# cyrillefavreau/Sol-R

Hardware: AMD Instinct MI355X
Metric: Mrays/s @1920x1080, 3-bounce Cornell (higher is better)
Workload: dtype f32; 1 GPU; cornell 1920x1080, 3 bounces + shadow rays, 75 boxes / 29 primitives, one GPU, whole frame; rays_per_frame=6518779, closest_hit_walks_rank0=3506171, lane_nodes=206382796, lane_prim_tests=37557299, wave_nodes=3396811, wave_prim_tests=626627, wave_walks=106204, cost_ordered_launch_rank0=True, frames_in_flight=3, setup_frames_before_warmup=48, frames_delivered=9105, order_free_nodes=46, short_ray_lists=1, gather=none (one GPU), strips=equal rows, parallelism=tile1

## Files before the change

sol-r_amd/csrc/engine.h:

```cpp
#ifndef SOLR_ENGINE_H
#define SOLR_ENGINE_H

#include <hip/hip_runtime.h>

#include <atomic>
#include <chrono>
#include <cstdio>
#include <cstdlib>
#include <cstring>
#include <string>
#include <utility>
#include <vector>

#include "../../include/solr_hip.h"
#include "renderer.h"
#include "lists_device.h"
#include "list_builders.h"

namespace solreng
{
struct HostProfile
{
    const bool on = getenv("SOLR_HIP_HOST_PROFILE") != nullptr;
    struct Entry
// ... 184 lines not shown
    VARIANT_AUTOMATIC = 0,
    VARIANT_EXACT_LIST = 3,
    VARIANT_ALL_FEATURES = 4,
    VARIANT_NO_GROUPING = 5,
    VARIANT_NO_ORDER_FREE = 6,
    VARIANT_STACK_IN_LDS = 7,
    VARIANT_REFERENCE_LEAVES = 8,
    VARIANT_AO_FIXED_STRIDE = 9,
    VARIANT_NAN_DEEP_STACK = 10,
    VARIANT_UNSORTED_LISTS = 12,
    VARIANT_NO_BAND_WORDS = 13,
    VARIANT_ZERO_STREAM_COUNTERS = 14,
    VARIANT_NO_LAMP_CUTOFF = 15,
    VARIANT_ALL_TRIPS = 16,
    VARIANT_UPLOADED_BUILD_BOXES = 17,
    VARIANT_UPLOADED_SPHERE_LEAVES = 18
};

__host__ __device__ inline int primitiveKind(int type, int facts)
{
    if (!(facts & PRIM_FAST0))
        return KIND_GENERAL;
    if (type == ptSphere && !(facts & PRIM_PROCEDURAL))
        return KIND_SPHERE;
    if ((type == ptXYPlane || type == ptYZPlane || type == ptXZPlane) && !(facts & (PRIM_TEXTURED | PRIM_WIRE2)) &&
        !(type == ptYZPlane && (facts & PRIM_EMISSIVE)))
        return type == ptXYPlane ? KIND_PLANE_XY : (type == ptYZPlane ? KIND_PLANE_YZ : KIND_PLANE_XZ);
    if (type == ptTriangle)
        return KIND_TRIANGLE;
    if (type == ptCylinder || type == ptCone)
        return KIND_CYLINDER;
// ... 33 lines not shown
        return features | F_PLANE;
    }
}

struct NodeList
{
    int copies, lists;
    explicit NodeList(int copies_ = 1, int lists_ = 1) : copies(copies_), lists(lists_) {}
    std::vector<float4> rows;
    std::vector<int> start, origin;
    int nb = 0;
    unsigned offRows = 0, offLeaf = 0;
    unsigned offStart = 0;
    int ordered = 0;
    bool tight = false;
    std::vector<int> refitLevels;

    void reset() { *this = NodeList(copies, lists); }
    unsigned nodes() const { return (unsigned)lists * (unsigned)nb; }
    unsigned rowsOf(int list) const { return solrdev::listRows(offRows, (unsigned)nb, (unsigned)list); }
    unsigned offThin() const { return solrdev::listThin(offRows, nodes()); }
    unsigned offSorted() const { return solrdev::listSorted(offRows, nodes()); }
    unsigned layRows(unsigned row)
    {
        offRows = row;
        return row + (unsigned)copies * solrdev::listCopyRows(nodes());
    }
    unsigned layStart(unsigned row)
    {
        offStart = row * 4;
        return row + (nodes() + 3u) / 4u;
    }
    unsigned layLeaf(unsigned row)
    {
        row = (row + 3u) & ~3u;
        offLeaf = row;
        return row + 4u * nodes() + 4u;
// ... 69 lines not shown
    int slotA, slotB;
    bool moves;
};
struct Morph
{
    MorphKey keys[MORPH_SLOTS];
    int nbTrackKeys = 0;
    std::vector<MorphLampAnswer> lampAnswers;
    long lampChecked = -1;
    DeviceBuffer lampFlag;
    int nbDeviceMorphs = 0;
    int nbDeviceTrackMorphs = 0;
};
struct Scene
{
    NodeList exact = NodeList(1, 1), walk = NodeList(2, 1), orderFree = NodeList(3, solrdev::ORDER_FREE_LISTS);
    std::vector<float4> hostPrims;
    int nbPrimitives = 0;
    DeviceBuffer lamps;
    int nbLamps = 0;
    int nested = 1;
    bool walkEncloses = false;
    OrderFreeState lists;
    Rotation rotation;
    Morph morph;
    long retags = 0;
    Arena arena;

    struct Served
    {
        int rotations, translations, lampMoves, edits, materialSets, morphs, trackMorphs;
// ... 559 lines not shown
void h2dMaterialsOne(Material *materials, int nbActiveMaterials);
MaterialRecord materialRecord(const Material &material, int i, solrdev::MaterialHot &hot, solrdev::MaterialCold &cold);
void h2dRandomsOne(float *randoms);
void h2dRandomsSizedOne(const float *randoms, long count);
void h2dTexturesOne(int activeTextures, TextureInfo *textureInfos);
void h2dLightInformationOne(LightInformation *lightInformation, int lightInformationSize);
void setMovableOne(const unsigned char *flags, int nbPrimitives);
void retagPrimitives();
void checkTextureTables();
void maybeBuildOrderFreeLists();
void flushGeometry();
void pullGeometry();
void ensureHostFreeLists();
void buildLeafRecords();
void tightenListsAgain();
float thinReachWanted(float viewDistance);
bool listEnclosesInArena(const NodeList &list);
ListKnobs listKnobs();
PruneDecider pruneDecider();
bool orderFreeListsUsable();
bool lampCutoffUsable();
bool shortRayListsChoice();
SceneArgs prepareScene(const SceneInfo &sceneInfo, bool exactNodes);
bool deepNodeList(const SceneArgs &S);
bool canRotateOne(const float center[3], const float cosAngles[3], const float sinAngles[3], float viewDistance,
                  const char *who = "solr_hip_rotate_primitives");
int rotatePrimitivesOne(const float center[3], const float cosAngles[3], const float sinAngles[3], float viewDistance);
bool refitMovedScene(float viewDistance);
void refreshExactList();
int setMorphKeysOne(const Primitive *first, const Primitive *last, int nbPrimitives);
// ... 75 lines not shown
```

sol-r_amd/csrc/renderer_kernel.h:

```cpp
#ifndef SOLR_RENDERER_KERNEL_H
#define SOLR_RENDERER_KERNEL_H

#include "renderer.h"

using namespace solrdev;

template <int COUNT, int FEAT, bool VOLUME = false>
#ifndef SOLR_GENERIC_WAVES
#define SOLR_GENERIC_WAVES 0
#endif
#ifndef SOLR_WAVES_PER_EU
#define SOLR_WAVES_PER_EU 4
#endif
__global__ __launch_bounds__(WAVE, (SOLR_GENERIC_WAVES && (FEAT & F_TEX)) ? SOLR_GENERIC_WAVES : SOLR_WAVES_PER_EU) void k_standardRenderer(const SceneArgs, const FrameArgs,
                                                           PixelRecord *__restrict__,
                                                           int4 *__restrict__, unsigned char *__restrict__,
                                                           unsigned long long *__restrict__)
{
    extern __shared__ float ldsStack[];
    constexpr int ARGS = FEAT | F_ARGS;
    constexpr int TRACE = (FEAT & (F_TRI | F_TEX)) ? FEAT : ARGS;
    const RendererArgs &A = rendererArgs();
    const FrameArgs &F = A.F;
    const Scene &S = A.scene();
// ... 402 lines not shown
    for (int j = 0; j < walks; ++j)
    {
        const int4 h = head[1 + j];
        const int kind = __builtin_amdgcn_readfirstlane(h.x);
        if (kind == WALK_GENERAL)
        {
            ++left_out;
            continue;
        }
        const float4 a = rays[((size_t)j * 64 + lane) * 2], b = rays[((size_t)j * 64 + lane) * 2 + 1];
        const int doneAfter = __float_as_int(b.w);
        const bool took_part = doneAfter >= 0;
        const WalkRay r = makeWalkRay(V(a.x, a.y, a.z), took_part ? V(b.x, b.y, b.z) : V(1.f, 1.f, 1.f));
        const int order = (FEAT & F_DEEP) ? (__builtin_amdgcn_readfirstlane(h.w) >> 1) & 3 : 0;
        const Scene W = walkList(S, __builtin_amdgcn_readfirstlane(h.y) != 0, __builtin_amdgcn_readfirstlane(h.z),
                                 (__builtin_amdgcn_readfirstlane(h.w) & 1) != 0, order != 0);
        const PackedRay pr = packRay(r);
        const float cutOff = a.w;
        int cursor = took_part ? 0 : SOLR_CURSOR_DONE;
        int cur = 0, visit = 0;
        while (cur < W.nbBoxes)
        {
            if (ballot(cursor != SOLR_CURSOR_DONE) == 0ull)
                break;
            int nbPrimitives;
            bool entered;
            int leaf;
            if ((FEAT & F_DEEP) && order == 1)
                leaf = advanceTidyDeepSorted(W, pr, cutOff, cursor, cur, nbPrimitives, entered);
            else if ((FEAT & F_DEEP) && order == 2)
                leaf = advanceTidyDeepReversed(W, pr, cutOff, cursor, cur, nbPrimitives, entered);
// ... 17 lines not shown
```

sol-r_amd/csrc/rt_device.h:

```cpp
#pragma once

#include <hip/hip_runtime.h>
#include "pow_table.h"

#include "../../include/solr_types.h"
#include "scene_layout.h"

namespace solrdev
{
#define SOLR_DEV __device__ __forceinline__

struct v3
{
    float x, y, z;
};

SOLR_DEV v3 V(float x, float y, float z)
{
    v3 r;
    r.x = x;
    r.y = y;
    r.z = z;
    return r;
}
// ... 856 lines not shown
    }
    return v;
}

#define SOLR_CURSOR_DONE 0x7fffffff

#define SOLR_WALK_SLOTS 16
#define SOLR_WALK_SLOT_BYTES (16 * (SOLR_WALK_SLOTS + 1) + SOLR_WALK_SLOTS * 64 * 32)
enum WalkKind
{
    WALK_CLOSEST = 0,
    WALK_SHADOW = 1,
    WALK_GENERAL = 2
};
SOLR_DEV void recordWalk(Counters &cnt, int kind, bool freeList, int octant, bool took_part, const WalkRay &r, float cutOff,
                         int doneAfter, bool tight = false, int order = 0)
{
    const unsigned j = cnt.ordinal++;
    if (j >= SOLR_WALK_SLOTS || !cnt.record)
        return;
    const int lane = (int)threadIdx.x & 63;
    float4 *lanes = (float4 *)(cnt.record + 16 * (SOLR_WALK_SLOTS + 1)) + ((size_t)j * 64 + lane) * 2;
    lanes[0] = make_float4(r.o.x, r.o.y, r.o.z, cutOff);
    lanes[1] = make_float4(r.d.x, r.d.y, r.d.z, __int_as_float(took_part ? doneAfter : -1));
    if (lane == 0)
        ((int4 *)cnt.record)[1 + j] = make_int4(kind, freeList ? 1 : 0, octant, (tight ? 1 : 0) | (order << 1));
}

template <int FEAT>
SOLR_DEV bool extendedGeometry(const SceneInfo &si);
struct PrimRec
{
    Row2 head;
    float4 c, d;
    int pi;
    bool packed;
};
SOLR_DEV bool planeClass(int type)
{
    return !(type == ptSphere || type == ptEnvironment || type == ptCylinder || type == ptCone || type == ptEllipsoid ||
             type == ptTriangle);
// ... 812 lines not shown
    int octant = 0;
    bool reversed = false;
    if (freeOrder)
    {
        const int signs = ((r.d.x < 0.f ? 1 : 0) | (r.d.y < 0.f ? 2 : 0) | (r.d.z < 0.f ? 4 : 0)) ^ 7;
        const int lane = (int)__builtin_ctzll(ballot(active));
        octant = __builtin_amdgcn_readlane(signs, lane);
        reversed = (FEAT & F_DEEP) && S.sortedLists && ballot(active && signs != octant) == 0ull;
    }
    if (freeOrder || lampCut)
        farFree = 1.0002f + 1.0e-4f * (fabsf(r.o.x) + fabsf(r.o.y) + fabsf(r.o.z)) / lengthOL;
    const float farOrdered =
        (lampCut && longRay(r.d) && minDistance >= 2.f) ? fminf(minDistance, farFree) : minDistance;
    const bool tight = (FEAT & F_PLANE) && tidy && S.tightLists && ballot(active && !tightRay(r, si)) == 0ull;
    reversed = reversed && !tight;
    const Scene W = walkList(S, freeOrder, octant, tight, reversed);
    const int nbBoxes = W.nbBoxes;
    const PackedRay pr = packRay(r);
    int cursor = (active && result < si.shadowIntensity) ? 0 : SOLR_CURSOR_DONE;
    const bool walked = cursor != SOLR_CURSOR_DONE;
    int visit = 0, doneAfter = SOLR_CURSOR_DONE;
    int cur = 0;
    Row2 node;
    node.a = node.b = make_float4(0.f, 0.f, 0.f, 0.f);
    if (!tidy)
        node = boxNode(S, 0);
    while (cur < nbBoxes)
    {
        if (ballot(cursor != SOLR_CURSOR_DONE) == 0ull)
            break;
        int leaf = cur, nbPrimitives;
// ... 131 lines not shown
                }
            }
        }
        if (COUNT == 2)
            ++visit;
        if (cursor != SOLR_CURSOR_DONE && !(result < si.shadowIntensity))
        {
            cursor = SOLR_CURSOR_DONE;
            if (COUNT == 2)
                doneAfter = visit;
        }
        SOLR_T(cnt.tLeaf += SOLR_NOW() - ta; ++cnt.nLeaf;)
    }
    if (COUNT == 2)
        recordWalk(cnt, tidy ? WALK_SHADOW : WALK_GENERAL, freeOrder, octant, walked, r, freeOrder ? farFree : farOrdered,
                   doneAfter, tight, reversed ? 2 : 0);
    result = fmaxf(0.f, fminf(result, si.shadowIntensity));
    SOLR_T(cnt.tShadow += SOLR_NOW() - tw0;)
    return result;
}


SOLR_DEV float rnd(const Scene &S, long i)
{
    return (i >= 0 && i < S.nbRandoms) ? S.randoms[i] : 0.f;
}

template <int FEAT>
SOLR_DEV float4 intersectionShader(const Scene &S, const SceneInfo &si, int pi, int type, int materialId,
                                   const MaterialHot &mh, v3 intersection, v3 areas, const TexOut &o)
{
// ... 979 lines not shown
```

sol-r_amd/csrc/scene_layout.h:

```cpp
#pragma once

#include <hip/hip_runtime.h>

namespace solrdev
{
struct alignas(16) MaterialHot
{
    float4 innerIllumination;
    float4 color;
    float4 specular;
    float reflection, refraction, transparency, opacity;
    int4 attributes;
    int4 ids;
};
static_assert(sizeof(MaterialHot) == 96, "MaterialHot");

struct alignas(16) MaterialCold
{
    int4 textureMapping;
    int4 textureOffset;
    int4 textureIds;
    int4 advancedTextureOffset;
    int4 advancedTextureIds;
    float2 mappingOffset;
// ... 42 lines not shown
    ROW_SIZE_MAT = 1,
    ROW_P1_INDEX = 2,
    ROW_P2 = 3,
    ROW_N0 = 4,
    ROW_N1 = 5,
    ROW_N2 = 6,
    ROW_UV = 7,
    PRIM_ROWS = 8
};

enum ShadowFacts
{
    SHADOWS_OPAQUE = 1,
    SHADOWS_LAMP_CUTOFF = 2,
    SHADOWS_ALL_TRIPS = 4
};

struct SceneArgs
{
    const void *geometry;
    const void *materials;
    const void *textures;
    const void *randoms;
    unsigned offBoxes, offBoxStart, offPrims, offLights, offMatCold;
    int nbBoxes;
    int nbPrimitives;
    int nbLights;
    int nbLamps;
    int nested;
    int orderedBoxes;
    long nbRandoms;
    unsigned offLeaf;
    unsigned offBoxesFree, offLeafFree;
    int nbBoxesFree;
    int opaqueShadows;
    int shortRayLists;
    int tightLists;
    int sortedLists;
};

const int ORDER_FREE_LISTS = 8;
__host__ __device__ constexpr unsigned listCopyRows(unsigned nodes) { return 2u * nodes + 2u; }
__host__ __device__ constexpr unsigned listRows(unsigned offRows, unsigned nb, unsigned list) { return offRows + 2u * (list * nb); }
__host__ __device__ constexpr unsigned listThin(unsigned offRows, unsigned nodes) { return offRows + listCopyRows(nodes); }
__host__ __device__ constexpr unsigned listSorted(unsigned offRows, unsigned nodes) { return offRows + 2u * listCopyRows(nodes); }
__host__ __device__ constexpr unsigned listLeaf(unsigned offLeaf, unsigned nb, unsigned list) { return offLeaf + 4u * (list * nb); }

#define SOLR_CONST_AS __attribute__((address_space(4)))
typedef float f4v __attribute__((ext_vector_type(4)));
typedef int i4v __attribute__((ext_vector_type(4)));
typedef const SOLR_CONST_AS f4v *cf4p;
typedef const SOLR_CONST_AS i4v *ci4p;
typedef const SOLR_CONST_AS int *cip;
typedef const SOLR_CONST_AS float *cfp;
typedef const SOLR_CONST_AS unsigned char *cbp;

struct Scene
{
    cf4p geo;
    cf4p mat;
// ... 34 lines not shown
    s.nbLamps = a.nbLamps;
    s.nested = a.nested;
    s.orderedBoxes = a.orderedBoxes;
    s.nbRandoms = a.nbRandoms;
    s.offLeaf = a.offLeaf;
    s.offBoxesFree = a.offBoxesFree;
    s.offLeafFree = a.offLeafFree;
    s.nbBoxesFree = a.nbBoxesFree;
    s.opaqueShadows = a.opaqueShadows;
    s.shortRayLists = a.shortRayLists;
    s.tightLists = a.tightLists;
    s.sortedLists = a.sortedLists;
    return s;
}

__device__ __forceinline__ Scene walkList(const Scene &S, bool freeList, int octant, bool thin, bool sorted)
{
    Scene W = S;
    unsigned nodes = (unsigned)S.nbBoxes;
    if (freeList)
    {
        nodes = (unsigned)ORDER_FREE_LISTS * (unsigned)S.nbBoxesFree;
        W.offBoxes = listRows(S.offBoxesFree, (unsigned)S.nbBoxesFree, (unsigned)octant);
        W.offLeaf = listLeaf(S.offLeafFree, (unsigned)S.nbBoxesFree, (unsigned)octant);
        W.nbBoxes = S.nbBoxesFree;
    }
    if (freeList && sorted)
    {
        W.offBoxes = listSorted(W.offBoxes, nodes);
        W.nbBoxes = S.nbBoxesFree << 5;
    }
    else if (thin)
        W.offBoxes = listThin(W.offBoxes, nodes);
    return W;
}

typedef float f8v __attribute__((ext_vector_type(8)));
typedef const SOLR_CONST_AS f8v *cf8p;
typedef const SOLR_CONST_AS char *ccp;

__device__ __forceinline__ float4 ld4(cf4p p, unsigned row)
{
    const f4v v = *(cf4p)((ccp)p + (row << 4));
    return make_float4(v.x, v.y, v.z, v.w);
}
struct Row2
{
    float4 a, b;
// ... 88 lines not shown
```

sol-r_amd/csrc/solr_arena.hip:

```cpp
#include <hip/hip_runtime.h>

#include <cmath>

#include "../../include/solr_hip.h"
#include "rt_device.h"

using namespace solrdev;

#include "renderer.h"
#include "engine.h"

using namespace solreng;

namespace solreng
{
__global__ __launch_bounds__(256) void k_buildLeafRecords(float4 *__restrict__ arena, unsigned offNodes, unsigned offStart,
                                                         unsigned offPrims, unsigned offLeaf, int nbNodes)
{
    const int i = blockIdx.x * blockDim.x + threadIdx.x;
    if (i >= nbNodes)
        return;
    float4 r0 = make_float4(0.f, 0.f, 0.f, 0.f), r1 = r0, r2 = r0, r3 = r0;
    const int nb = __float_as_int(arena[offNodes + 2u * (unsigned)i + 1u].z);
    if (nb > 0)
// ... 59 lines not shown
    for (int j = i + 1; j < end; ++j)
    {
        const float4 b = arena[offTight + 2u * (unsigned)j + 1u];
        if (__float_as_int(b.z) <= 0)
            continue;
        const float4 a = arena[offTight + 2u * (unsigned)j];
        lx = fminf(lx, a.x), ly = fminf(ly, a.y), lz = fminf(lz, a.z);
        hx = fmaxf(hx, b.x), hy = fmaxf(hy, b.y), hz = fmaxf(hz, a.w);
    }
    const float nlx = fmaxf(row0.x, lx), nly = fmaxf(row0.y, ly), nlz = fmaxf(row0.z, lz);
    const float nhx = fminf(row1.x, hx), nhy = fminf(row1.y, hy), nhz = fminf(row0.w, hz);
    if (!(nlx <= nhx && nly <= nhy && nlz <= nhz))
        return;
    arena[offTight + 2u * (unsigned)i] = make_float4(nlx, nly, nlz, nhz);
    arena[offTight + 2u * (unsigned)i + 1u] = make_float4(nhx, nhy, row1.z, row1.w);
}

__global__ __launch_bounds__(256) void k_listEncloses(const float4 *__restrict__ arena, unsigned offNodes, unsigned offStart,
                                                      unsigned offPrims, int nbNodes, int nbPrims, int *bad)
{
    const int i = blockIdx.x * blockDim.x + threadIdx.x;
    if (i >= nbNodes)
        return;
    const float4 a = arena[offNodes + 2u * (unsigned)i], b = arena[offNodes + 2u * (unsigned)i + 1u];
    const int count = __float_as_int(b.z);
    const int end = min(i + max(__float_as_int(b.w), 1), nbNodes);
    bool encloses = true;
    if (count <= 0)
    {
        for (int j = i + 1; j < end && encloses;)
// ... 105 lines not shown
    static const bool off = getenv("SOLR_HIP_NO_TIGHT_LEAVES") != nullptr;
    const int nbNodes = (int)list.nodes(), listLength = list.nb;
    const bool worth = g.facts.plainPlanes || (g.facts.looseSpheres && (g.facts.sceneFeatures & F_PLANE) != 0);
    if (off || !worth || nbNodes <= 0 || listLength <= 0 || listLength > 65536 || !ok())
        return false;
    float4 *arena = (float4 *)g.scene.arena.geometry.ptr;
    const float margin = g.facts.sceneExtent * (1.f / 1024.f);
    const dim3 grid((unsigned)((nbNodes + 255) / 256));
    hipLaunchKernelGGL(k_tightenLeaves, grid, dim3(256), 0, sceneStream(), arena, list.offRows, list.offThin(), list.offStart, g.scene.arena.offPrims,
                       nbNodes, margin, g.facts.thinReach);
    hipLaunchKernelGGL(k_tightenInner, grid, dim3(256), 0, sceneStream(), arena, list.offThin(), nbNodes, listLength);
    HIPCHECK(hipGetLastError());
    return ok();
}

__global__ __launch_bounds__(256) void k_sortNodeBounds(float4 *__restrict__ arena, unsigned offBoxesFree, unsigned offSorted, int nb)
{
    const int i = blockIdx.x * blockDim.x + threadIdx.x;
    if (i > 8 * nb)
        return;
    float4 a = make_float4(0.f, 0.f, 0.f, 0.f), b = a;
    if (i < 8 * nb)
    {
        const int octant = i / nb;
        a = arena[offBoxesFree + 2u * (unsigned)i];
        b = arena[offBoxesFree + 2u * (unsigned)i + 1u];
        if (octant & 1)
        {
            const float t = a.x;
            a.x = b.x;
// ... 26 lines not shown
    hipLaunchKernelGGL(k_sortNodeBounds, dim3((unsigned)((8 * list.nb + 1 + 255) / 256)), dim3(256), 0, sceneStream(),
                       (float4 *)g.scene.arena.geometry.ptr, list.offRows, list.offSorted(), list.nb);
    HIPCHECK(hipGetLastError());
    return ok();
}

static void deriveList(NodeList &list)
{
    const bool orderFree = &list == &g.scene.orderFree;
    const int n = (orderFree && g.scene.lists.freeStale) ? 0 : (int)list.nodes();
    if (n > 0)
        hipLaunchKernelGGL(k_buildLeafRecords, dim3((unsigned)((n + 255) / 256)), dim3(256), 0, sceneStream(), (float4 *)g.scene.arena.geometry.ptr,
                           list.offRows, list.offStart, g.scene.arena.offPrims, list.offLeaf, n);
    HIPCHECK(hipGetLastError());
    list.tight = list.copies > 1 && n > 0 && tightenList(list);
    if (orderFree)
        g.scene.lists.sortedFree = n > 0 && sortFreeLists();
}

void buildLeafRecords()
{
    if (!ok() || !g.scene.arena.geometry.ptr)
        return;
    for (NodeList *list : {&g.scene.exact, &g.scene.walk, &g.scene.orderFree})
        deriveList(*list);
    HIPCHECK(hipStreamSynchronize(sceneStream()));
}

void tightenListsAgain()
{
    if (!ok() || !g.scene.arena.geometry.ptr)
        return;
    for (NodeList *list : {&g.scene.walk, &g.scene.orderFree})
        if (list->tight)
            list->tight = tightenList(*list);
    HIPCHECK(hipStreamSynchronize(sceneStream()));
}

static void copyStagedLists()
{
    const NodeList &list = g.scene.orderFree;
    char *arena = (char *)g.scene.arena.geometry.ptr;
    const SolrDeviceLists &stage = g.scene.lists.freeStage;
    HIPCHECK(hipMemcpyAsync(arena + (size_t)list.offRows * 16, stage.rows, (size_t)list.nodes() * 32, hipMemcpyDeviceToDevice, sceneStream()));
    HIPCHECK(hipMemcpyAsync(arena + (size_t)list.offStart * 4, stage.start, (size_t)list.nodes() * 4, hipMemcpyDeviceToDevice, sceneStream()));
}

static void appendFreeLists()
{
    const unsigned end = g.scene.orderFree.layLeaf(g.scene.orderFree.layStart(g.scene.orderFree.layRows(g.scene.arena.rowsFixed)));
// ... 210 lines not shown
    return g.scene.orderFree.nb > 0 && g.facts.primsContained && !g.scene.lists.freeStale && g.scene.nested && g.scene.walk.ordered &&
           g.variant != VARIANT_NO_ORDER_FREE;
}

bool lampCutoffUsable()
{
    return g.scene.walkEncloses && g.facts.primsContained && g.scene.nested && g.scene.walk.ordered && g.variant != VARIANT_NO_LAMP_CUTOFF;
}

static int tightListsFor(const SceneArgs &S, const SceneInfo &sceneInfo, bool exactNodes)
{
    if (exactNodes || g.variant == VARIANT_REFERENCE_LEAVES || !g.scene.walk.tight || !g.scene.walkEncloses || !sceneInfo.extendedGeometry)
        return 0;
    if (S.nbBoxesFree > 0 && !g.scene.orderFree.tight)
        return 0;
    return (sceneInfo.viewDistance > 0.f && sceneInfo.viewDistance <= 64.f * g.facts.sceneExtent) ? 1 : 0;
}

static bool sortedListsUsable(int nbBoxesFree)
{
    return nbBoxesFree > 0 && g.scene.lists.sortedFree && g.variant != VARIANT_UNSORTED_LISTS;
}

bool shortRayListsChoice()
{
    static const int fromEnv = getenv("SOLR_HIP_SHORT_RAY_LISTS") ? atoi(getenv("SOLR_HIP_SHORT_RAY_LISTS")) : -1;
    const int mode = g.shortRayListsMode >= 0 ? g.shortRayListsMode : fromEnv;
    return mode < 0 ? activeFlights() >= 2 : mode != 0;
}

static SceneArgs makeScene(bool exactNodes)
// ... 67 lines not shown
```

sol-r_amd/csrc/solr_diag.hip:

```cpp
#include <hip/hip_runtime.h>
#include <dlfcn.h>
#include <fcntl.h>
#include <sched.h>
#include <sys/mman.h>
#include <sys/stat.h>
#include <unistd.h>

#include <atomic>

#include <cmath>
#include <cstdio>
#include <cstdlib>
#include <cstring>
#include <string>
#include <functional>
#include <chrono>
#include <vector>

#include "../../include/solr_hip.h"
#include "rt_device.h"
#include "device_pool.h"
#include "lists_device.h"

using namespace solrdev;
// ... 61 lines not shown
    }
    HIPCHECK(hipMemcpyAsync(bitmapOut, bitmap, pixels * SOLR_COLOR_DEPTH, hipMemcpyDeviceToHost, stream));
    HIPCHECK(hipStreamSynchronize(stream));
    return ok() ? 0 : -1;
}

void lastFrame(int out[6])
{
    memcpy(out, g.lastFrame, sizeof(g.lastFrame));
}

int listCopy(int list, int what, void *out, int capacity)
{
    if (!ready("solr_hip_probe_list_copy"))
        return -1;
    ARGCHECK(list >= 0 && list <= 2 && what >= 0 && what <= 4, "solr_hip_probe_list_copy: no such list or copy");
    ARGCHECK(g.scene.arena.geometry.ptr != nullptr || g.scene.arena.geometryDirty, "solr_hip_probe_list_copy: no scene uploaded");
    if (!ok())
        return -1;
    HIPCHECK(hipSetDevice(g.device));
    flushGeometry();
    if (list == 1)
        refreshExactList();
    quiesce();
    if (!ok() || !g.scene.arena.geometry.ptr)
        return -1;
    const NodeList &L = list == 0 ? g.scene.walk : (list == 1 ? g.scene.exact : g.scene.orderFree);
    const unsigned nodes = (list == 2 && g.scene.lists.freeStale) ? 0u : L.nodes();
    size_t at = 0, count = 0, unit = 16;
    switch (what)
    {
    case 0:
        at = (size_t)L.offRows * 16, count = 2 * (size_t)nodes;
        break;
    case 1:
        at = (size_t)L.offThin() * 16, count = (L.copies > 1 && L.tight) ? 2 * (size_t)nodes : 0;
        break;
    case 2:
        at = (size_t)L.offSorted() * 16, count = (list == 2 && L.copies > 2 && g.scene.lists.sortedFree) ? 2 * (size_t)nodes + 2 : 0;
        break;
    case 3:
        at = (size_t)L.offLeaf * 16, count = 4 * (size_t)nodes;
        break;
    default:
        at = (size_t)L.offStart * 4, count = nodes, unit = 4;
        break;
    }
    if (nodes == 0)
        count = 0;
    if (!out)
        return (int)count;
    ARGCHECK(count <= (size_t)(capacity < 0 ? 0 : capacity), "solr_hip_probe_list_copy: capacity too small");
    ARGCHECK(at + count * unit <= g.scene.arena.geometry.bytes, "solr_hip_probe_list_copy: the copy lies outside the arena");
    if (!ok())
        return -1;
    if (count)
        HIPCHECK(hipMemcpy(out, (const char *)g.scene.arena.geometry.ptr + at, count * unit, hipMemcpyDeviceToHost));
    return ok() ? (int)count : -1;
}

int walkOffer(const SceneInfo &sceneInfo, bool exactNodes, int out[8])
{
    SceneArgs S;
    int features, deep;
    hipStream_t stream;
    if (residentScene(sceneInfo, exactNodes, &S, &features, &deep, &stream) != 0)
        return -1;
    const float margin = g.facts.sceneExtent * (1.f / 1024.f), extent = g.facts.sceneExtent;
    out[0] = S.tightLists, out[1] = S.sortedLists, out[2] = S.nbBoxesFree, out[3] = S.opaqueShadows, out[4] = S.shortRayLists;
    out[5] = S.nbBoxes;
    memcpy(&out[6], &margin, 4);
    memcpy(&out[7], &extent, 4);
    return 0;
}
}

extern "C" {
static unsigned long long walkLists[6];
void solr_hip_walk_bound_lists(unsigned long long out[6])
{
    if (out)
        memcpy(out, walkLists, sizeof(walkLists));
}

// ... 393 lines not shown
```

sol-r_amd/csrc/solr_materials.hip:

```cpp
#include <hip/hip_runtime.h>

#include "../../include/solr_hip.h"
#include "rt_device.h"

using namespace solrdev;

#include "renderer.h"
#include "engine.h"

using namespace solreng;

namespace solreng
{
__global__ __launch_bounds__(256) void k_setPrimitiveMaterials(float4 *__restrict__ arena, unsigned offPrims, int nbPrimitives,
                                                               const int4 *__restrict__ batch, int nbRecords, int noKinds)
{
    const int e = blockIdx.x * blockDim.x + threadIdx.x;
    if (e >= nbRecords)
        return;
    const int4 r = batch[e];
    const int slot = r.x;
    if (slot < 0 || slot >= nbPrimitives)
        return;
    float4 *rows = arena + offPrims + (size_t)PRIM_ROWS * slot;
// ... 121 lines not shown
    HIPCHECK(hipMemcpyAsync(g.scene.rotation.materialSets.ptr, batch.data(), batch.size() * sizeof(int4), hipMemcpyHostToDevice, sceneStream()));
    hipLaunchKernelGGL(k_setPrimitiveMaterials, dim3((unsigned)((n + 255) / 256)), dim3(256), 0, sceneStream(),
                       (float4 *)g.scene.arena.geometry.ptr, g.scene.arena.offPrims, g.scene.nbPrimitives,
                       (const int4 *)g.scene.rotation.materialSets.ptr, n, general ? 1 : 0);
    LeafMaterialsFollow M;
    const int nodes = leafRecordsOfLists(g.scene, M.list);
    M.offPrims = g.scene.arena.offPrims;
    M.nbPrimitives = g.scene.nbPrimitives;
    if (nodes > 0)
        hipLaunchKernelGGL(k_followLeafRecords, dim3((unsigned)((nodes + 255) / 256)), dim3(256), 0, sceneStream(),
                           (float4 *)g.scene.arena.geometry.ptr, M);
    HIPCHECK(hipGetLastError());
    HIPCHECK(hipStreamSynchronize(sceneStream()));
    if (ok())
    {
        for (int i = 0; i < n; ++i)
        {
            float4 *r = &g.scene.hostPrims[(size_t)PRIM_ROWS * slots[i]];
            const int tag = bitsi(r[ROW_P0_TYPE].w), type = tag & PRIM_TYPE_MASK, facts = batch[(size_t)i].z;
            g.facts.count(type, factsOfTag(tag), -1);
            g.facts.count(type, facts, +1);
            r[ROW_P0_TYPE].w = bitsf(primitiveTag(type, facts, general));
            r[ROW_SIZE_MAT].w = bitsf(materialIds[i]);
            r[ROW_P2].w = bitsf(batch[(size_t)i].w);
        }
        g.facts.deriveFromCounts();
        g.scene.retagged();
    }
    g.scene.materialSetsServed(ok());
    return ok() ? 1 : 0;
}

enum
{
    RETAG_LINEAR = 8
};
__global__ __launch_bounds__(256) void k_retagMaterials(float4 *__restrict__ arena, unsigned offPrims, int nbPrimitives,
                                                        const int4 *__restrict__ batch, int nbRecords, int noKinds)
{
    const int p = blockIdx.x * blockDim.x + threadIdx.x;
    if (p >= nbPrimitives)
        return;
// ... 171 lines not shown
                               (const int4 *)M.editBatch.ptr, (int)plan.batch.size(), general ? 1 : 0);
            LeafMaterialsFollow F;
            const int nodes = leafRecordsOfLists(g.scene, F.list);
            F.offPrims = g.scene.arena.offPrims;
            F.nbPrimitives = g.scene.nbPrimitives;
            if (nodes > 0)
                hipLaunchKernelGGL(k_followLeafRecords, dim3((unsigned)((nodes + 255) / 256)), dim3(256), 0, sceneStream(),
                                   (float4 *)g.scene.arena.geometry.ptr, F);
            HIPCHECK(hipGetLastError());
        }
    }
    HIPCHECK(hipStreamSynchronize(sceneStream()));
    M.nbImaged = ok() ? M.nbImaged : -1;
    if (!ok())
        return 0;
    for (size_t k = 0; k < plan.ids.size(); ++k)
    {
        const size_t id = (size_t)plan.ids[k];
        M.imageHot[id] = plan.hot[k];
        M.imageCold[id] = plan.cold[k];
        M.materialTags[id] = plan.records[k].facts;
        M.materialAverage[id] = plan.records[k].average;
    }
    std::vector<TextureUse> uses;
    size_t k = 0;
    for (const TextureUse &use : M.textureUses)
    {
        for (; k < plan.ids.size() && plan.ids[k] < use.material; ++k)
            if (plan.records[k].textured)
                uses.push_back(plan.records[k].use);
// ... 14 lines not shown
            changedAt[(size_t)plan.batch[e].x] = (int)e;
        for (int p = 0; p < g.scene.nbPrimitives; ++p)
        {
            float4 *r = &g.scene.hostPrims[(size_t)PRIM_ROWS * p];
            const int material = bitsi(r[ROW_SIZE_MAT].w);
            if (material < 0 || material >= M.nbImaged || changedAt[(size_t)material] < 0)
                continue;
            const int4 &record = plan.batch[(size_t)changedAt[(size_t)material]];
            r[ROW_P0_TYPE].w = bitsf(primitiveTag(bitsi(r[ROW_P0_TYPE].w) & PRIM_TYPE_MASK, record.y, general));
            r[ROW_P2].w = bitsf(record.z);
        }
        g.facts = plan.after;
        g.scene.retagged();
        ++M.nbDeviceRetags;
    }
    ++M.nbDeviceEdits;
    return 1;
}

}

extern "C" {
int solr_hip_device_material_sets(void)
{
    return g.scene.rotation.nbDeviceMaterialSets;
}
int solr_hip_device_material_edits(void)
{
    return g.materials.nbDeviceEdits;
}
// ... 6 lines not shown
```

sol-r_amd/csrc/solr_probes.hip:

```cpp
#include <hip/hip_runtime.h>

#include <cstdio>
#include <cstring>
#include <string>
#include <vector>

#include "../../include/solr_hip.h"
#include "../../include/solr_hip_probes.h"
#include "../../include/solr_hip_probes_morph.h"
#include "rt_device.h"
#include "renderer.h"
#include "list_builders.h"
#include "lists_device.h"

using namespace solrdev;

namespace solrprobe
{
int residentScene(const SceneInfo &sceneInfo, bool exactNodes, SceneArgs *S, int *features, int *deepList, hipStream_t *stream);
void fail(int code, const char *what);
int ticketOfSerial(long long serial, int *slot, long long *period);
long long imageSerial(long long setTo);
int postProcess(const SceneInfo &sceneInfo, const PostProcessingInfo &ppInfo, const PostProcessingBuffer *frame,
                unsigned char *bitmapOut);
// ... 205 lines not shown
    const int e = blockIdx.x * 64 + threadIdx.x;
    const bool active = e < n;
    const int q = active ? e : 0;
    Counters cnt;
    memset(&cnt, 0, sizeof(cnt));
    float value = 0.f;
    v3 tint = V(0.f, 0.f, 0.f);
    unsigned long long todo = ballot(active);
    while (todo)
    {
        const int first = (int)__builtin_ctzll(todo);
        const int lamp = __builtin_amdgcn_readlane(lightId[q], first);
        const int it = __builtin_amdgcn_readlane(iteration[q], first);
        const bool lanes = active && lightId[q] == lamp && iteration[q] == it;
        v3 c = V(0.f, 0.f, 0.f);
        const float s = shadowWalk<false, FEAT>(S, si, lanes, at3(lampCenters, q), at3(origins, q), lamp, it, c, objectId[q], cnt);
        if (lanes)
        {
            value = s;
            tint = c;
        }
        todo &= ~ballot(lanes);
    }
    if (active)
    {
        result[e] = value;
        put3(color, e, tint);
    }
}

template <int FEAT>
// ... 741 lines not shown
```

Measured before the change: 31600 Mrays/s.

## Add shadow-specific thin BVH copy that culls lamp-only and non-fast leaves

Builds a third copy of the walk node list for shadow rays. Leaves whose primitives are all non-FAST0 or are the single lamp itself get an unenterable corner box, and inner bounds are re-tightened over the remaining leaves. Shadow walks select this copy through a new TIGHT_SHADOW_COPY bit, which is meant to avoid node and primitive tests that cannot occlude. The cost is extra arena rows, two build kernels, a rebuild whenever materials change FAST0, and added correctness complexity around lamp identity.

```diff
diff --git a/sol-r_amd/csrc/engine.h b/sol-r_amd/csrc/engine.h
--- a/sol-r_amd/csrc/engine.h
+++ b/sol-r_amd/csrc/engine.h
@@ -222,7 +222,8 @@
     VARIANT_NO_LAMP_CUTOFF = 15,
     VARIANT_ALL_TRIPS = 16,
     VARIANT_UPLOADED_BUILD_BOXES = 17,
-    VARIANT_UPLOADED_SPHERE_LEAVES = 18
+    VARIANT_UPLOADED_SPHERE_LEAVES = 18,
+    VARIANT_THIN_SHADOW_WALKS = 19
 };
 
 __host__ __device__ inline int primitiveKind(int type, int facts)
@@ -286,6 +287,7 @@
     unsigned offStart = 0;
     int ordered = 0;
     bool tight = false;
+    bool shadow = false;
     std::vector<int> refitLevels;
 
     void reset() { *this = NodeList(copies, lists); }
@@ -293,6 +295,7 @@
     unsigned rowsOf(int list) const { return solrdev::listRows(offRows, (unsigned)nb, (unsigned)list); }
     unsigned offThin() const { return solrdev::listThin(offRows, nodes()); }
     unsigned offSorted() const { return solrdev::listSorted(offRows, nodes()); }
+    unsigned offShadow() const { return solrdev::listShadow(offRows, nodes()); }
     unsigned layRows(unsigned row)
     {
         offRows = row;
@@ -392,7 +395,7 @@
 };
 struct Scene
 {
-    NodeList exact = NodeList(1, 1), walk = NodeList(2, 1), orderFree = NodeList(3, solrdev::ORDER_FREE_LISTS);
+    NodeList exact = NodeList(1, 1), walk = NodeList(3, 1), orderFree = NodeList(3, solrdev::ORDER_FREE_LISTS);
     std::vector<float4> hostPrims;
     int nbPrimitives = 0;
     DeviceBuffer lamps;
@@ -982,6 +985,7 @@
 void ensureHostFreeLists();
 void buildLeafRecords();
 void tightenListsAgain();
+void shadowListAgain();
 float thinReachWanted(float viewDistance);
 bool listEnclosesInArena(const NodeList &list);
 ListKnobs listKnobs();
diff --git a/sol-r_amd/csrc/renderer_kernel.h b/sol-r_amd/csrc/renderer_kernel.h
--- a/sol-r_amd/csrc/renderer_kernel.h
+++ b/sol-r_amd/csrc/renderer_kernel.h
@@ -440,7 +440,8 @@
         const WalkRay r = makeWalkRay(V(a.x, a.y, a.z), took_part ? V(b.x, b.y, b.z) : V(1.f, 1.f, 1.f));
         const int order = (FEAT & F_DEEP) ? (__builtin_amdgcn_readfirstlane(h.w) >> 1) & 3 : 0;
         const Scene W = walkList(S, __builtin_amdgcn_readfirstlane(h.y) != 0, __builtin_amdgcn_readfirstlane(h.z),
-                                 (__builtin_amdgcn_readfirstlane(h.w) & 1) != 0, order != 0);
+                                 (__builtin_amdgcn_readfirstlane(h.w) & 1) != 0, order != 0,
+                                 (__builtin_amdgcn_readfirstlane(h.w) & 8) != 0 ? 2u : 1u);
         const PackedRay pr = packRay(r);
         const float cutOff = a.w;
         int cursor = took_part ? 0 : SOLR_CURSOR_DONE;
diff --git a/sol-r_amd/csrc/rt_device.h b/sol-r_amd/csrc/rt_device.h
--- a/sol-r_amd/csrc/rt_device.h
+++ b/sol-r_amd/csrc/rt_device.h
@@ -894,7 +894,7 @@
     WALK_GENERAL = 2
 };
 SOLR_DEV void recordWalk(Counters &cnt, int kind, bool freeList, int octant, bool took_part, const WalkRay &r, float cutOff,
-                         int doneAfter, bool tight = false, int order = 0)
+                         int doneAfter, bool tight = false, int order = 0, bool shadowCopy = false)
 {
     const unsigned j = cnt.ordinal++;
     if (j >= SOLR_WALK_SLOTS || !cnt.record)
@@ -904,7 +904,7 @@
     lanes[0] = make_float4(r.o.x, r.o.y, r.o.z, cutOff);
     lanes[1] = make_float4(r.d.x, r.d.y, r.d.z, __int_as_float(took_part ? doneAfter : -1));
     if (lane == 0)
-        ((int4 *)cnt.record)[1 + j] = make_int4(kind, freeList ? 1 : 0, octant, (tight ? 1 : 0) | (order << 1));
+        ((int4 *)cnt.record)[1 + j] = make_int4(kind, freeList ? 1 : 0, octant, (tight ? 1 : 0) | (order << 1) | (shadowCopy ? 8 : 0));
 }
 
 template <int FEAT>
@@ -1747,7 +1747,8 @@
         (lampCut && longRay(r.d) && minDistance >= 2.f) ? fminf(minDistance, farFree) : minDistance;
     const bool tight = (FEAT & F_PLANE) && tidy && S.tightLists && ballot(active && !tightRay(r, si)) == 0ull;
     reversed = reversed && !tight;
-    const Scene W = walkList(S, freeOrder, octant, tight, reversed);
+    const unsigned thinCopy = (FEAT & F_PLANE) ? ((unsigned)S.tightLists + 1u) >> 1 : 1u;
+    const Scene W = walkList(S, freeOrder, octant, tight, reversed, thinCopy);
     const int nbBoxes = W.nbBoxes;
     const PackedRay pr = packRay(r);
     int cursor = (active && result < si.shadowIntensity) ? 0 : SOLR_CURSOR_DONE;
@@ -1909,7 +1910,7 @@
     }
     if (COUNT == 2)
         recordWalk(cnt, tidy ? WALK_SHADOW : WALK_GENERAL, freeOrder, octant, walked, r, freeOrder ? farFree : farOrdered,
-                   doneAfter, tight, reversed ? 2 : 0);
+                   doneAfter, tight, reversed ? 2 : 0, tight && !freeOrder && thinCopy == 2u);
     result = fmaxf(0.f, fminf(result, si.shadowIntensity));
     SOLR_T(cnt.tShadow += SOLR_NOW() - tw0;)
     return result;
diff --git a/sol-r_amd/csrc/scene_layout.h b/sol-r_amd/csrc/scene_layout.h
--- a/sol-r_amd/csrc/scene_layout.h
+++ b/sol-r_amd/csrc/scene_layout.h
@@ -80,6 +80,12 @@
     SHADOWS_OPAQUE = 1,
     SHADOWS_LAMP_CUTOFF = 2,
     SHADOWS_ALL_TRIPS = 4
+};
+
+enum TightLists
+{
+    TIGHT_LISTS = 1,
+    TIGHT_SHADOW_COPY = 2
 };
 
 struct SceneArgs
@@ -110,6 +116,8 @@
 __host__ __device__ constexpr unsigned listRows(unsigned offRows, unsigned nb, unsigned list) { return offRows + 2u * (list * nb); }
 __host__ __device__ constexpr unsigned listThin(unsigned offRows, unsigned nodes) { return offRows + listCopyRows(nodes); }
 __host__ __device__ constexpr unsigned listSorted(unsigned offRows, unsigned nodes) { return offRows + 2u * listCopyRows(nodes); }
+__host__ __device__ constexpr unsigned listShadow(unsigned offRows, unsigned nodes) { return offRows + 2u * listCopyRows(nodes); }
+#define SOLR_UNENTERABLE_CORNER 0x1p100f
 __host__ __device__ constexpr unsigned listLeaf(unsigned offLeaf, unsigned nb, unsigned list) { return offLeaf + 4u * (list * nb); }
 
 #define SOLR_CONST_AS __attribute__((address_space(4)))
@@ -174,7 +182,7 @@
     return s;
 }
 
-__device__ __forceinline__ Scene walkList(const Scene &S, bool freeList, int octant, bool thin, bool sorted)
+__device__ __forceinline__ Scene walkList(const Scene &S, bool freeList, int octant, bool thin, bool sorted, unsigned thinCopy = 1u)
 {
     Scene W = S;
     unsigned nodes = (unsigned)S.nbBoxes;
@@ -191,7 +199,7 @@
         W.nbBoxes = S.nbBoxesFree << 5;
     }
     else if (thin)
-        W.offBoxes = listThin(W.offBoxes, nodes);
+        W.offBoxes += (freeList ? 1u : thinCopy) * listCopyRows(nodes);
     return W;
 }
 
diff --git a/sol-r_amd/csrc/solr_arena.hip b/sol-r_amd/csrc/solr_arena.hip
--- a/sol-r_amd/csrc/solr_arena.hip
+++ b/sol-r_amd/csrc/solr_arena.hip
@@ -97,6 +97,85 @@
         return;
     arena[offTight + 2u * (unsigned)i] = make_float4(nlx, nly, nlz, nhz);
     arena[offTight + 2u * (unsigned)i + 1u] = make_float4(nhx, nhy, row1.z, row1.w);
+}
+
+__device__ __forceinline__ bool unenterable(const float4 &row0, const float4 &row1)
+{
+    const float c = SOLR_UNENTERABLE_CORNER;
+    return row0.x == c && row0.y == c && row0.z == c && row0.w == c && row1.x == c && row1.y == c;
+}
+__global__ __launch_bounds__(256) void k_shadowLeaves(float4 *__restrict__ arena, unsigned offThin, unsigned offShadow, unsigned offStart,
+                                                     unsigned offPrims, unsigned offLights, int nbNodes, int nbPrims, int nbLamps,
+                                                     int nbLights)
+{
+    const int i = blockIdx.x * blockDim.x + threadIdx.x;
+    if (i >= nbNodes)
+        return;
+    float4 row0 = arena[offThin + 2u * (unsigned)i], row1 = arena[offThin + 2u * (unsigned)i + 1u];
+    const int nb = __float_as_int(row1.z);
+    if (nb > 0)
+    {
+        bool oneLamp = nbLamps == 1 && nbLights >= 1;
+        const int lamp = nbLights >= 1 ? __float_as_int(arena[offLights].w) : 0;
+        for (int l = 1; l < nbLights && oneLamp; ++l)
+            oneLamp = __float_as_int(arena[offLights + 3u * (unsigned)l].w) == lamp;
+        const int start = ((const int *)arena)[offStart + (unsigned)i];
+        bool counts = start < 0 || (long long)start + nb > nbPrims;
+        for (int k = 0; k < nb && !counts; ++k)
+        {
+            const float4 *prim = arena + offPrims + (size_t)PRIM_ROWS * (size_t)(start + k);
+            const int tag = __float_as_int(prim[ROW_P0_TYPE].w), index = __float_as_int(prim[ROW_P1_INDEX].w);
+            counts = (tag & PRIM_FAST0) != 0 && !(oneLamp && index == lamp);
+        }
+        if (!counts)
+        {
+            const float c = SOLR_UNENTERABLE_CORNER;
+            row0 = make_float4(c, c, c, c);
+            row1 = make_float4(c, c, row1.z, row1.w);
+        }
+    }
+    arena[offShadow + 2u * (unsigned)i] = row0;
+    arena[offShadow + 2u * (unsigned)i + 1u] = row1;
+}
+
+__global__ __launch_bounds__(256) void k_shadowInner(float4 *__restrict__ arena, unsigned offShadow, int nbNodes)
+{
+    const int i = blockIdx.x * blockDim.x + threadIdx.x;
+    if (i >= nbNodes)
+        return;
+    const float4 row0 = arena[offShadow + 2u * (unsigned)i], row1 = arena[offShadow + 2u * (unsigned)i + 1u];
+    const int nb = __float_as_int(row1.z), skip = __float_as_int(row1.w);
+    if (nb > 0 || skip <= 1)
+        return;
+    const int end = min(i + skip, nbNodes);
+    float lx = INFINITY, ly = INFINITY, lz = INFINITY, hx = -INFINITY, hy = -INFINITY, hz = -INFINITY;
+    bool leaves = false, enterable = false;
+    for (int j = i + 1; j < end; ++j)
+    {
+        const float4 b = arena[offShadow + 2u * (unsigned)j + 1u];
+        if (__float_as_int(b.z) <= 0)
+            continue;
+        const float4 a = arena[offShadow + 2u * (unsigned)j];
+        leaves = true;
+        if (unenterable(a, b))
+            continue;
+        enterable = true;
+        lx = fminf(lx, a.x), ly = fminf(ly, a.y), lz = fminf(lz, a.z);
+        hx = fmaxf(hx, b.x), hy = fmaxf(hy, b.y), hz = fmaxf(hz, a.w);
+    }
+    if (!leaves)
+        return;
+    const float c = SOLR_UNENTERABLE_CORNER;
+    float nlx = c, nly = c, nlz = c, nhx = c, nhy = c, nhz = c;
+    if (enterable)
+    {
+        nlx = fmaxf(row0.x, lx), nly = fmaxf(row0.y, ly), nlz = fmaxf(row0.z, lz);
+        nhx = fminf(row1.x, hx), nhy = fminf(row1.y, hy), nhz = fminf(row0.w, hz);
+        if (!(nlx <= nhx && nly <= nhy && nlz <= nhz))
+            return;
+    }
+    arena[offShadow + 2u * (unsigned)i] = make_float4(nlx, nly, nlz, nhz);
+    arena[offShadow + 2u * (unsigned)i + 1u] = make_float4(nhx, nhy, row1.z, row1.w);
 }
 
 __global__ __launch_bounds__(256) void k_listEncloses(const float4 *__restrict__ arena, unsigned offNodes, unsigned offStart,
@@ -232,6 +311,48 @@
     return ok();
 }
 
+static bool shadowLeafOnHost(const NodeList &list)
+{
+    const size_t n = list.nodes(), nbPrims = g.scene.hostPrims.size() / PRIM_ROWS;
+    const size_t nbLights = std::min((size_t)std::max(g.lights.nbLights, 0), g.lights.hostLights.size() / 3);
+    if (list.rows.size() < 2 * n || list.start.size() < n)
+        return false;
+    bool oneLamp = g.scene.nbLamps == 1 && nbLights >= 1;
+    const int lamp = nbLights >= 1 ? bitsi(g.lights.hostLights[0].w) : 0;
+    for (size_t l = 1; l < nbLights && oneLamp; ++l)
+        oneLamp = bitsi(g.lights.hostLights[3 * l].w) == lamp;
+    for (size_t i = 0; i < n; ++i)
+    {
+        const int nb = bitsi(list.rows[2 * i + 1].z), start = list.start[i];
+        if (nb <= 0)
+            continue;
+        bool counts = start < 0 || (size_t)start + (size_t)nb > nbPrims;
+        for (int k = 0; k < nb && !counts; ++k)
+        {
+            const float4 *prim = &g.scene.hostPrims[(size_t)PRIM_ROWS * (size_t)(start + k)];
+            counts = (bitsi(prim[ROW_P0_TYPE].w) & PRIM_FAST0) != 0 && !(oneLamp && bitsi(prim[ROW_P1_INDEX].w) == lamp);
+        }
+        if (!counts)
+            return true;
+    }
+    return false;
+}
+
+static bool shadowList(const NodeList &list)
+{
+    const int nbNodes = (int)list.nodes();
+    if (list.copies < 3 || list.lists != 1 || nbNodes <= 0 || !ok())
+        return false;
+    float4 *arena = (float4 *)g.scene.arena.geometry.ptr;
+    const dim3 grid((unsigned)((nbNodes + 255) / 256));
+    hipLaunchKernelGGL(k_shadowLeaves, grid, dim3(256), 0, sceneStream(), arena, list.offThin(), list.offShadow(), list.offStart,
+                       g.scene.arena.offPrims, g.scene.arena.offLights, nbNodes, (int)(g.scene.hostPrims.size() / PRIM_ROWS), g.scene.nbLamps,
+                       (int)std::min((size_t)std::max(g.lights.nbLights, 0), g.lights.hostLights.size() / 3));
+    hipLaunchKernelGGL(k_shadowInner, grid, dim3(256), 0, sceneStream(), arena, list.offShadow(), nbNodes);
+    HIPCHECK(hipGetLastError());
+    return ok() && shadowLeafOnHost(list);
+}
+
 __global__ __launch_bounds__(256) void k_sortNodeBounds(float4 *__restrict__ arena, unsigned offBoxesFree, unsigned offSorted, int nb)
 {
     const int i = blockIdx.x * blockDim.x + threadIdx.x;
@@ -288,6 +409,7 @@
                            list.offRows, list.offStart, g.scene.arena.offPrims, list.offLeaf, n);
     HIPCHECK(hipGetLastError());
     list.tight = list.copies > 1 && n > 0 && tightenList(list);
+    list.shadow = &list == &g.scene.walk && list.tight && shadowList(list);
     if (orderFree)
         g.scene.lists.sortedFree = n > 0 && sortFreeLists();
 }
@@ -308,6 +430,15 @@
     for (NodeList *list : {&g.scene.walk, &g.scene.orderFree})
         if (list->tight)
             list->tight = tightenList(*list);
+    g.scene.walk.shadow = g.scene.walk.tight && shadowList(g.scene.walk);
+    HIPCHECK(hipStreamSynchronize(sceneStream()));
+}
+
+void shadowListAgain()
+{
+    if (!ok() || !g.scene.arena.geometry.ptr)
+        return;
+    g.scene.walk.shadow = g.scene.walk.tight && shadowList(g.scene.walk);
     HIPCHECK(hipStreamSynchronize(sceneStream()));
 }
 
@@ -548,7 +679,10 @@
         return 0;
     if (S.nbBoxesFree > 0 && !g.scene.orderFree.tight)
         return 0;
-    return (sceneInfo.viewDistance > 0.f && sceneInfo.viewDistance <= 64.f * g.facts.sceneExtent) ? 1 : 0;
+    if (!(sceneInfo.viewDistance > 0.f && sceneInfo.viewDistance <= 64.f * g.facts.sceneExtent))
+        return 0;
+    const bool shadowCopy = g.scene.walk.shadow && g.variant != VARIANT_THIN_SHADOW_WALKS && sceneInfo.viewDistance <= 0x1p50f;
+    return TIGHT_LISTS | (shadowCopy ? TIGHT_SHADOW_COPY : 0);
 }
 
 static bool sortedListsUsable(int nbBoxesFree)
diff --git a/sol-r_amd/csrc/solr_diag.hip b/sol-r_amd/csrc/solr_diag.hip
--- a/sol-r_amd/csrc/solr_diag.hip
+++ b/sol-r_amd/csrc/solr_diag.hip
@@ -99,7 +99,7 @@
 {
     if (!ready("solr_hip_probe_list_copy"))
         return -1;
-    ARGCHECK(list >= 0 && list <= 2 && what >= 0 && what <= 4, "solr_hip_probe_list_copy: no such list or copy");
+    ARGCHECK(list >= 0 && list <= 2 && what >= 0 && what <= 5, "solr_hip_probe_list_copy: no such list or copy");
     ARGCHECK(g.scene.arena.geometry.ptr != nullptr || g.scene.arena.geometryDirty, "solr_hip_probe_list_copy: no scene uploaded");
     if (!ok())
         return -1;
@@ -127,6 +127,9 @@
     case 3:
         at = (size_t)L.offLeaf * 16, count = 4 * (size_t)nodes;
         break;
+    case 5:
+        at = (size_t)L.offShadow() * 16, count = (list == 0 && L.copies > 2 && L.tight && L.shadow) ? 2 * (size_t)nodes : 0;
+        break;
     default:
         at = (size_t)L.offStart * 4, count = nodes, unit = 4;
         break;
@@ -152,7 +155,7 @@
     if (residentScene(sceneInfo, exactNodes, &S, &features, &deep, &stream) != 0)
         return -1;
     const float margin = g.facts.sceneExtent * (1.f / 1024.f), extent = g.facts.sceneExtent;
-    out[0] = S.tightLists, out[1] = S.sortedLists, out[2] = S.nbBoxesFree, out[3] = S.opaqueShadows, out[4] = S.shortRayLists;
+    out[0] = S.tightLists & TIGHT_LISTS, out[1] = S.sortedLists, out[2] = S.nbBoxesFree, out[3] = S.opaqueShadows, out[4] = S.shortRayLists;
     out[5] = S.nbBoxes;
     memcpy(&out[6], &margin, 4);
     memcpy(&out[7], &extent, 4);
diff --git a/sol-r_amd/csrc/solr_materials.hip b/sol-r_amd/csrc/solr_materials.hip
--- a/sol-r_amd/csrc/solr_materials.hip
+++ b/sol-r_amd/csrc/solr_materials.hip
@@ -159,10 +159,12 @@
     HIPCHECK(hipStreamSynchronize(sceneStream()));
     if (ok())
     {
+        bool fast0Moved = false;
         for (int i = 0; i < n; ++i)
         {
             float4 *r = &g.scene.hostPrims[(size_t)PRIM_ROWS * slots[i]];
             const int tag = bitsi(r[ROW_P0_TYPE].w), type = tag & PRIM_TYPE_MASK, facts = batch[(size_t)i].z;
+            fast0Moved = fast0Moved || ((tag ^ facts) & PRIM_FAST0) != 0;
             g.facts.count(type, factsOfTag(tag), -1);
             g.facts.count(type, facts, +1);
             r[ROW_P0_TYPE].w = bitsf(primitiveTag(type, facts, general));
@@ -171,6 +173,8 @@
         }
         g.facts.deriveFromCounts();
         g.scene.retagged();
+        if (fast0Moved)
+            shadowListAgain();
     }
     g.scene.materialSetsServed(ok());
     return ok() ? 1 : 0;
@@ -372,6 +376,9 @@
     M.nbImaged = ok() ? M.nbImaged : -1;
     if (!ok())
         return 0;
+    bool fast0Moved = false;
+    for (const int4 &record : plan.batch)
+        fast0Moved = fast0Moved || ((record.y ^ factsOfMaterial(record.x)) & PRIM_FAST0) != 0;
     for (size_t k = 0; k < plan.ids.size(); ++k)
     {
         const size_t id = (size_t)plan.ids[k];
@@ -416,6 +423,12 @@
         g.scene.retagged();
         ++M.nbDeviceRetags;
     }
+    if (fast0Moved)
+    {
+        shadowListAgain();
+        if (!ok())
+            return 0;
+    }
     ++M.nbDeviceEdits;
     return 1;
 }
diff --git a/sol-r_amd/csrc/solr_probes.hip b/sol-r_amd/csrc/solr_probes.hip
--- a/sol-r_amd/csrc/solr_probes.hip
+++ b/sol-r_amd/csrc/solr_probes.hip
@@ -243,7 +243,10 @@
         const int it = __builtin_amdgcn_readlane(iteration[q], first);
         const bool lanes = active && lightId[q] == lamp && iteration[q] == it;
         v3 c = V(0.f, 0.f, 0.f);
-        const float s = shadowWalk<false, FEAT>(S, si, lanes, at3(lampCenters, q), at3(origins, q), lamp, it, c, objectId[q], cnt);
+        Scene Sq = S;
+        if (S.nbLights < 1 || lamp != asint(loadLight(S, 0).location.w))
+            Sq.tightLists &= ~TIGHT_SHADOW_COPY;
+        const float s = shadowWalk<false, FEAT>(Sq, si, lanes, at3(lampCenters, q), at3(origins, q), lamp, it, c, objectId[q], cnt);
         if (lanes)
         {
             value = s;
```

After: 32000 Mrays/s (median of 6 runs). 1.01x the previous value.
